# gmh14/tssplat

Hardware: NVIDIA H100
Metric: geometry_energy_grad_iters_per_sec_64x4k (higher is better)
Workload: dtype f32

## Files before the change

include/tssplat_b200.h:

```cpp
#ifndef TSSPLAT_B200_H_
#define TSSPLAT_B200_H_

#include <stdint.h>

#ifdef __cplusplus
extern "C" {
#endif

#define TSB_VERSION 2

enum {
  TSB_OK = 0,
  TSB_E_INVALID = -1,
  TSB_E_MESH = -2,
  TSB_E_CUDA = -3,
  TSB_E_NOMEM = -4
};

typedef struct tsb_handle_s *tsb_handle_t;

typedef struct {
  int32_t warps_per_cta;
  int32_t laplacian_scale;
  int32_t ring_slots;
  int32_t force_global;
  int32_t tet_cost_x100;
  int32_t enable_amips;
  int32_t reserved[2];
} tsb_options_t;

typedef struct {
  float c1, c2;
  int32_t order;
  float c3;
  int32_t reserved[4];
} tsb_terms_t;

typedef struct {
  int32_t n;
  int32_t nele;
  int32_t n_components;
  int32_t grid;
  int32_t warps_per_cta;
  int32_t ctas_per_sm;
  int32_t mode_global;
  int32_t smem_bytes;
  int32_t ring_slots;
  int32_t n_segments;
  int32_t n_boundary_faces;
  int32_t max_component_vertices;
  int64_t nnz;
  int64_t nnz_padded;
  int64_t device_bytes;
  int64_t stream_bytes;
} tsb_info_t;

int tsb_create(const float *rest_xyz, const int32_t *tets, int32_t n, int32_t nele,
               const tsb_options_t *opt, int device, tsb_handle_t *out);

void tsb_destroy(tsb_handle_t h);

const char *tsb_last_error(tsb_handle_t h);

int tsb_get_info(tsb_handle_t h, tsb_info_t *info);

int tsb_energy_grad(tsb_handle_t h, const float *x_dev, float c1, float c2, int32_t order,
                    float gradH, const float *gradH_dev, float *energy_out_dev,
                    float *grad_out_dev, void *stream);

int tsb_energy_grad_ex(tsb_handle_t h, const float *x_dev, const tsb_terms_t *terms, float gradH,
                       const float *gradH_dev, float *energy_out_dev, float *grad_out_dev, void *stream);

int tsb_energy_grad_host(tsb_handle_t h, const float *x_host, float c1, float c2, int32_t order,
                         float gradH, float *energy_out_host, float *grad_out_host, void *stream);

int tsb_scale(const float *g_dev, int64_t count, float gradH, const float *gradH_dev,
              float *out_dev, void *stream);

int tsb_grad_limit(float *grad_dev, int64_t count, float s_threshold, float s, float *work_dev, void *stream);

int tsb_adam_uniform_step(float *p_dev, const float *grad_dev, float *g1_dev, float *g2_dev,
                          int64_t count, double lr, double beta1, double beta2, int32_t step,
                          double grad_limit, float *work_dev, void *stream);

typedef struct tsb_surface_s *tsb_surface_t;
int tsb_surface_create(const int32_t *surface_vid, int32_t nsv, const int32_t *surface_f, int32_t nsf,
                       int32_t n_tet_vertices, int device, tsb_surface_t *out);
void tsb_surface_destroy(tsb_surface_t s);
const char *tsb_surface_last_error(tsb_surface_t s);
int tsb_surface_forward(tsb_surface_t s, const float *tet_v_dev, float *v_pos_dev, float *v_nrm_dev, void *stream);
int tsb_surface_backward(tsb_surface_t s, const float *tet_v_dev, const float *grad_v_pos_dev,
                         const float *grad_v_nrm_dev, float *grad_tet_v_dev, void *stream);

int tsb_surface_extract(const int32_t *tets_host, int32_t nele, int32_t n, int device, int32_t *nsv_out,
                        int32_t *nsf_out, int32_t **surface_vid_out, int32_t **surface_f_out);
void tsb_free_host(void *p);
const char *tsb_setup_last_error(void);

#ifdef __cplusplus
}
#endif
#endif
```

tssplat_b200/_capi.py:

```python
from __future__ import annotations

import ctypes as C
import os

from . import build as _build

LIB_PATH = os.environ.get("TSSPLAT_B200_LIB") or _build.LIB_PATH

TSB_OK, TSB_E_INVALID, TSB_E_MESH, TSB_E_CUDA, TSB_E_NOMEM = 0, -1, -2, -3, -4

EXPORTED_SYMBOLS = (
    "tsb_create", "tsb_destroy", "tsb_last_error", "tsb_get_info", "tsb_energy_grad", "tsb_energy_grad_ex", "tsb_energy_grad_host", "tsb_scale",
    "tsb_grad_limit", "tsb_adam_uniform_step",
    "tsb_surface_create", "tsb_surface_destroy", "tsb_surface_last_error", "tsb_surface_forward", "tsb_surface_backward",
    "tsb_surface_extract", "tsb_free_host", "tsb_setup_last_error",
)


class tsb_options_t(C.Structure):
    _fields_ = [("warps_per_cta", C.c_int32), ("laplacian_scale", C.c_int32), ("ring_slots", C.c_int32),
                ("force_global", C.c_int32), ("tet_cost_x100", C.c_int32), ("enable_amips", C.c_int32), ("reserved", C.c_int32 * 2)]


class tsb_terms_t(C.Structure):
    _fields_ = [("c1", C.c_float), ("c2", C.c_float), ("order", C.c_int32), ("c3", C.c_float), ("reserved", C.c_int32 * 4)]


class tsb_info_t(C.Structure):
    _fields_ = [
        ("n", C.c_int32), ("nele", C.c_int32), ("n_components", C.c_int32), ("grid", C.c_int32),
        ("warps_per_cta", C.c_int32), ("ctas_per_sm", C.c_int32), ("mode_global", C.c_int32),
        ("smem_bytes", C.c_int32), ("ring_slots", C.c_int32), ("n_segments", C.c_int32),
        ("n_boundary_faces", C.c_int32), ("max_component_vertices", C.c_int32),
        ("nnz", C.c_int64), ("nnz_padded", C.c_int64), ("device_bytes", C.c_int64), ("stream_bytes", C.c_int64),
    ]


def _load() -> C.CDLL:
    if not os.path.exists(LIB_PATH):
        raise ImportError(
            f"{LIB_PATH} is missing: the CUDA library has not been built "
            "(run `python -m tssplat_b200.build`); tssplat_b200 has no CPU fallback")
    try:
        lib = C.CDLL(LIB_PATH)
    except OSError as e:
        raise ImportError(f"cannot load {LIB_PATH}: {e}; tssplat_b200 has no CPU fallback") from e
    vp, f32, i32, i64 = C.c_void_p, C.c_float, C.c_int32, C.c_int64
    lib.tsb_create.restype = C.c_int
    lib.tsb_create.argtypes = [vp, vp, i32, i32, C.POINTER(tsb_options_t), C.c_int, C.POINTER(vp)]
    lib.tsb_destroy.restype = None
    lib.tsb_destroy.argtypes = [vp]
    lib.tsb_last_error.restype = C.c_char_p
    lib.tsb_last_error.argtypes = [vp]
    lib.tsb_get_info.restype = C.c_int
    lib.tsb_get_info.argtypes = [vp, C.POINTER(tsb_info_t)]
    lib.tsb_energy_grad.restype = C.c_int
    lib.tsb_energy_grad.argtypes = [vp, vp, f32, f32, i32, f32, vp, vp, vp, vp]
    lib.tsb_energy_grad_ex.restype = C.c_int
    lib.tsb_energy_grad_ex.argtypes = [vp, vp, C.POINTER(tsb_terms_t), f32, vp, vp, vp, vp]
    lib.tsb_energy_grad_host.restype = C.c_int
    lib.tsb_energy_grad_host.argtypes = [vp, vp, f32, f32, i32, f32, vp, vp, vp]
    lib.tsb_scale.restype = C.c_int
    lib.tsb_scale.argtypes = [vp, i64, f32, vp, vp, vp]
    lib.tsb_grad_limit.restype = C.c_int
    lib.tsb_grad_limit.argtypes = [vp, i64, f32, f32, vp, vp]
    lib.tsb_adam_uniform_step.restype = C.c_int
    lib.tsb_adam_uniform_step.argtypes = [vp, vp, vp, vp, i64, C.c_double, C.c_double, C.c_double, i32, C.c_double, vp, vp]
    lib.tsb_surface_create.restype = C.c_int
    lib.tsb_surface_create.argtypes = [vp, i32, vp, i32, i32, C.c_int, C.POINTER(vp)]
    lib.tsb_surface_destroy.restype = None
    lib.tsb_surface_destroy.argtypes = [vp]
    lib.tsb_surface_last_error.restype = C.c_char_p
    lib.tsb_surface_last_error.argtypes = [vp]
    lib.tsb_surface_forward.restype = C.c_int
    lib.tsb_surface_forward.argtypes = [vp, vp, vp, vp, vp]
    lib.tsb_surface_backward.restype = C.c_int
    lib.tsb_surface_backward.argtypes = [vp, vp, vp, vp, vp, vp]
    lib.tsb_surface_extract.restype = C.c_int
    lib.tsb_surface_extract.argtypes = [vp, C.c_int32, C.c_int32, C.c_int, C.POINTER(C.c_int32), C.POINTER(C.c_int32),
                                        C.POINTER(C.POINTER(C.c_int32)), C.POINTER(C.POINTER(C.c_int32))]
    lib.tsb_free_host.restype = None
    lib.tsb_free_host.argtypes = [vp]
    lib.tsb_setup_last_error.restype = C.c_char_p
    lib.tsb_setup_last_error.argtypes = []
    return lib


# ... 13 lines not shown
```

tssplat_b200/csrc/tsb_capi.cu:

```cuda
#include <cuda_runtime.h>

#include <cstdio>
#include <cstring>
#include <string>
#include <vector>

#include "../../include/tssplat_b200.h"
#include "tsb_kernels.cuh"
#include "tsb_plan.h"

struct tsb_handle_s {
  int device = 0;
  tsb::KParams kp{};
  tsb::LaunchConfig lc{};
  float *stage_x[2] = {nullptr, nullptr}, *stage_grad[2] = {nullptr, nullptr}, *stage_energy[2] = {nullptr, nullptr};
  cudaStream_t s_pipe[2] = {nullptr, nullptr};
  cudaEvent_t ev_run[2] = {nullptr, nullptr}, ev_done[2] = {nullptr, nullptr};
  unsigned host_calls = 0;
  bool amips = false;
  tsb_info_t info{};
  std::vector<void *> allocs;
  std::string err;
};

// ... 97 lines not shown
  pc.grid_cb = [&](int area_verts, bool &global_mode, int &grid, std::string &err) -> int {
    if (!global_mode) {
      int r = ring;
      while (r > 2 && tsb::energy_smem_bytes(nw, r, cpc, area_verts, false) > smem_optin) --r;
      if (tsb::energy_smem_bytes(nw, r, cpc, area_verts, false) > smem_optin) global_mode = true;
      else slots = r;
    }
    if (global_mode) while (slots > 2 && tsb::energy_smem_bytes(nw, slots, cpc, 0, true) > smem_optin) --slots;
    smem = tsb::energy_smem_bytes(nw, slots, cpc, global_mode ? 0 : area_verts, global_mode);
    int ctas = 0;
    cudaError_t e = tsb::energy_occupancy(nw, smem, global_mode, pc.enable_amips != 0, &ctas);
    if (e != cudaSuccess || ctas < 1) {
      err = std::string("kernel does not fit the device: ") + (e != cudaSuccess ? cudaGetErrorString(e) : "occupancy 0");
      return TSB_E_CUDA;
    }
    ctas_per_sm = std::min(ctas, nw == 16 ? 1 : 2);
    grid = ctas_per_sm * sms;
    return TSB_OK;
  };

  tsb::HostPlan plan;
  std::string err;
  int rc = tsb::build_plan(rest_xyz, tets, n, nele, pc, plan, err);
  if (rc != TSB_OK) return fail(nullptr, rc, err);

  tsb_handle_t h = new tsb_handle_s();
  h->device = device;
  tsb::KParams &kp = h->kp;
#define TSB_TRY(expr) do { rc = (expr); if (rc != TSB_OK) { g_create_err = h->err; tsb_destroy(h); return rc; } } while (0)
  TSB_TRY(upload(h, plan.stream, kp.stream, 16));
  TSB_TRY(upload(h, plan.X4, kp.X4, 4));
  TSB_TRY(upload(h, plan.segs, kp.segs));
  TSB_TRY(upload(h, plan.cta_seg, kp.cta_seg, 2));
  TSB_TRY(upload(h, plan.wdesc, kp.wdesc, 2));
  TSB_TRY(upload(h, plan.wseg, kp.wseg, 2));
  TSB_TRY(upload(h, plan.vlist, kp.vlist));
  TSB_TRY(upload(h, plan.pos16, kp.pos16, 2));
  TSB_TRY(upload(h, plan.pos_gid, kp.pos_gid));
  TSB_TRY(upload(h, plan.orphans, kp.orphans));
  if (pc.enable_amips) {
    TSB_TRY(upload(h, plan.Bt, kp.Bt, 4));
    TSB_TRY(upload(h, plan.wtc0, kp.wtc0));
  }
  TSB_TRY(alloc_zero(h, size_t(plan.n_components), &kp.done));
  TSB_TRY(upload(h, std::vector<unsigned long long>(size_t(plan.grid) * 4, tsb::kEnergySentinel), kp.cta_energy, 2));
#ifdef TSB_TRACE
  TSB_TRY(alloc_zero(h, size_t(plan.grid) * 16, &kp.trace));
#endif
  if (plan.mode_global) {
    TSB_TRY(alloc_zero(h, size_t(plan.n), &kp.u4g));
    TSB_TRY(alloc_zero(h, size_t(plan.n), &kp.x4g));
  }
#undef TSB_TRY
  kp.n_orphans = int32_t(plan.orphans.size());
  kp.n_components = plan.n_components;
  kp.n = plan.n;
  kp.vh = plan.vh;
  kp.ring_bytes = tsb::energy_ring_bytes(slots, cpc, plan.mode_global != 0);
  kp.cells_per_chunk = cpc;
  kp.ring_slots = slots;
  kp.stage_bytes = plan.mode_global ? 0 : plan.area_verts * 32;
  h->lc = tsb::LaunchConfig{nw, plan.grid, smem, plan.mode_global, 0};
  h->amips = pc.enable_amips != 0;

  tsb_info_t &I = h->info;
  I.n = plan.n; I.nele = plan.nele; I.n_components = plan.n_components; I.grid = plan.grid;
  I.warps_per_cta = nw; I.ctas_per_sm = ctas_per_sm; I.mode_global = plan.mode_global; I.smem_bytes = smem;
  I.ring_slots = slots; I.n_segments = int32_t(plan.segs.size()); I.n_boundary_faces = plan.n_boundary_faces;
  I.max_component_vertices = plan.max_comp_verts; I.nnz = plan.nnz; I.nnz_padded = plan.nnz_padded;
  int64_t staged = 0;
  for (const tsb::SegHdr &s : plan.segs) staged += s.nv;
  I.stream_bytes = int64_t(plan.stream.size()) + (plan.mode_global ? int64_t(plan.n) * (12 + 16 + 64) : staged * (16 + 12 + 2)) +
                   int64_t(plan.n) * 12 + int64_t(plan.segs.size()) * 32 + int64_t(plan.grid) * (16 + 8 * nw);
  *out = h;
  return TSB_OK;
}

void tsb_destroy(tsb_handle_t h) {
  if (!h) return;
  DeviceGuard guard(h->device);
  for (int k = 0; k < 2; ++k) {
    if (h->ev_run[k]) cudaEventDestroy(h->ev_run[k]);
    if (h->ev_done[k]) cudaEventDestroy(h->ev_done[k]);
    if (h->s_pipe[k]) cudaStreamDestroy(h->s_pipe[k]);
  }
  for (void *p : h->allocs) cudaFree(p);
  delete h;
}

const char *tsb_last_error(tsb_handle_t h) { return h ? h->err.c_str() : g_create_err.c_str(); }

int tsb_get_info(tsb_handle_t h, tsb_info_t *info) {
  if (!h || !info) return TSB_E_INVALID;
  *info = h->info;
  return TSB_OK;
}

static int energy_grad_impl(tsb_handle_t h, const float *x_dev, float c1, float c2, float c3, int32_t order, float gradH,
                            const float *gradH_dev, float *energy_out_dev, int energy4, float *grad_out_dev, void *stream) {
  if (!h) return TSB_E_INVALID;
  if (!x_dev || !energy_out_dev) return fail(h, TSB_E_INVALID, "x_dev and energy_out_dev must be non-null");
  if (order != 2 && order != 4)
    return fail(h, TSB_E_INVALID, "order must be 2 or 4 (the reference yields zeros for anything else: tet_spheres_cuda.cu:57-63)");
  if (c3 != 0.f && !h->amips) return fail(h, TSB_E_INVALID, "c3 != 0 needs a handle created with tsb_options_t.enable_amips = 1");
  DeviceGuard guard(h->device);
  if (!guard.ok) return fail(h, TSB_E_CUDA, "cannot select the handle's CUDA device");
  tsb::KParams kp = h->kp;
  kp.x = x_dev; kp.grad = grad_out_dev; kp.energy_out = energy_out_dev; kp.gradH_dev = gradH_dev;
  kp.c1 = c1; kp.c2 = c2; kp.c3 = c3; kp.gradH = gradH; kp.order = order; kp.energy4 = energy4;
  tsb::LaunchConfig lc = h->lc;
  lc.amips = c3 != 0.f ? 1 : 0;
  cudaError_t e = tsb::launch_energy_grad(kp, lc, static_cast<cudaStream_t>(stream));
  if (e != cudaSuccess) return fail(h, TSB_E_CUDA, std::string("energy_grad launch: ") + cudaGetErrorString(e));
  return TSB_OK;
}

int tsb_energy_grad(tsb_handle_t h, const float *x_dev, float c1, float c2, int32_t order, float gradH,
                    const float *gradH_dev, float *energy_out_dev, float *grad_out_dev, void *stream) {
  return energy_grad_impl(h, x_dev, c1, c2, 0.f, order, gradH, gradH_dev, energy_out_dev, 0, grad_out_dev, stream);
}

int tsb_energy_grad_ex(tsb_handle_t h, const float *x_dev, const tsb_terms_t *terms, float gradH, const float *gradH_dev,
                       float *energy_out_dev, float *grad_out_dev, void *stream) {
  if (!h) return TSB_E_INVALID;
  if (!terms) return fail(h, TSB_E_INVALID, "terms is null");
  return energy_grad_impl(h, x_dev, terms->c1, terms->c2, terms->c3, terms->order, gradH, gradH_dev, energy_out_dev, 1, grad_out_dev, stream);
// ... 110 lines not shown
```

tssplat_b200/csrc/tsb_kernels.cu:

```cuda
#include <cuda_runtime.h>

#include <cmath>
#include <cstdint>

#include "tsb_kernels.cuh"

namespace tsb {

namespace {

__device__ __forceinline__ double warp_sum(double v) {
#pragma unroll
  for (int o = 16; o > 0; o >>= 1) v += __shfl_xor_sync(0xffffffffu, v, o);
  return v;
}

__device__ __forceinline__ uint32_t smem_u32(const void *p) { return uint32_t(__cvta_generic_to_shared(p)); }
__device__ __forceinline__ void mbar_fence_init() { asm volatile("fence.mbarrier_init.release.cluster;" ::: "memory"); }
__device__ __forceinline__ unsigned int ld_acquire(const unsigned int *p) {
  unsigned int v;
  asm volatile("ld.acquire.gpu.global.u32 %0, [%1];" : "=r"(v) : "l"(p) : "memory");
  return v;
}

constexpr int align_up(int v, int a) { return (v + a - 1) / a * a; }
constexpr int kMaxSlots = 8;
constexpr unsigned long long kSentinel = kEnergySentinel;

#ifdef TSB_TRACE
__device__ __forceinline__ unsigned long long gtime() { unsigned long long t; asm volatile("mov.u64 %0, %%globaltimer;" : "=l"(t)); return t; }
#define TSB_STAMP(i) do { if (tid == 0 && p.trace) p.trace[blockIdx.x * 16 + (i)] = (i) == 0 ? gtime() : (unsigned long long)clock64(); } while (0)
#else
#define TSB_STAMP(i) do { } while (0)
#endif

__host__ __device__ constexpr int off_rings(int stage_bytes) { return align_up(stage_bytes, 128); }
__host__ __device__ constexpr int off_bars(int stage_bytes, int nw, int ring) { return off_rings(stage_bytes) + nw * ring; }
__host__ __device__ constexpr int off_red(int stage_bytes, int nw, int ring) { return off_bars(stage_bytes, nw, ring) + nw * kMaxSlots * 8; }
constexpr int kSegTab = 16;
__host__ __device__ constexpr int off_segtab(int stage_bytes, int nw, int ring) { return align_up(off_red(stage_bytes, nw, ring) + nw * 24, 32); }
__host__ __device__ constexpr int off_wsegtab(int stage_bytes, int nw, int ring) { return off_segtab(stage_bytes, nw, ring) + kSegTab * 32; }
__host__ __device__ constexpr int smem_total(int stage_bytes, int nw, int ring) { return align_up(off_wsegtab(stage_bytes, nw, ring) + kSegTab * nw * 4, 128); }

struct f32x2 { float lo, hi; };
__device__ __forceinline__ f32x2 pk2(float lo, float hi) { return f32x2{lo, hi}; }
__device__ __forceinline__ float sum2(f32x2 v) { return v.lo + v.hi; }
__device__ __forceinline__ void fma2_acc(f32x2 &acc, f32x2 a, f32x2 b) { acc.lo = fmaf(a.lo, b.lo, acc.lo); acc.hi = fmaf(a.hi, b.hi, acc.hi); }

__device__ __forceinline__ float rel_u(float x, float X, float c) {
  const float s = x - X, bb = s - x;
  const float e = (x - (s - bb)) + (-X - bb);
  return (s - c) + e;
}

template <bool GLOBAL> struct Fmt;
template <> struct Fmt<false> { static constexpr uint32_t CELL = kCellStaged, IB = 2, TPL = 2; };
template <> struct Fmt<true> { static constexpr uint32_t CELL = kCellGlobal, IB = 4, TPL = 1; };

template <uint32_t CELL>
struct WarpStream {
  const unsigned char *next_src;
  uint32_t bytes_left;
  uint32_t bars;
  unsigned char *ring;
  unsigned char *cell;
  uint32_t chunk_bytes, cpc, nslot;
  uint32_t cc, slot, phase, cells_left;
  int lane;

  __device__ __forceinline__ void request(uint32_t smem_dst, uint32_t bar) {
    const uint32_t bytes = min(chunk_bytes, bytes_left);
    asm volatile("mbarrier.arrive.expect_tx.shared::cta.b64 _, [%0], %1;" ::"r"(bar), "r"(bytes) : "memory");
    asm volatile("cp.async.bulk.shared::cluster.global.mbarrier::complete_tx::bytes [%0], [%1], %2, [%3];" ::"r"(smem_dst), "l"(next_src),
                 "r"(bytes), "r"(bar)
                 : "memory");
    next_src += bytes;
    bytes_left -= bytes;
  }
  __device__ __forceinline__ void wait(uint32_t bar, uint32_t parity) {
    uint32_t ok;
    do {
      asm volatile("{\n.reg .pred p;\nmbarrier.try_wait.parity.shared::cta.b64 p, [%1], %2;\nselp.u32 %0, 1, 0, p;\n}" : "=r"(ok) : "r"(bar), "r"(parity) : "memory");
    } while (!ok);
  }
  __device__ __forceinline__ void begin() {
    if (cells_left) wait(bars, 0);
  }
  __device__ __forceinline__ uint32_t avail() const { return cpc - cc; }
  __device__ __forceinline__ void advance(uint32_t n) {
    cell += n * CELL;
    cc += n;
    cells_left -= n;
    if (cc == cpc) {
      cc = 0;
      __syncwarp();
      if (lane == 0 && bytes_left) request(smem_u32(cell) - chunk_bytes, bars + slot * 8);
      if (++slot == nslot) { slot = 0; cell = ring; phase ^= 1u; }
      if (cells_left) wait(bars + slot * 8, phase);
    }
  }
};

template <int NW, int MINB, bool GLOBAL, bool AMIPS>
__global__ void __launch_bounds__(NW * 32, MINB) energy_grad_kernel(const KParams p) {
  using F = Fmt<GLOBAL>;
  constexpr int NT = NW * 32;
  constexpr uint32_t CELL = F::CELL, WOFF = 128 * F::IB;
  constexpr int SV = GLOBAL ? 1 : (1024 + NT - 1) / NT;
  extern __shared__ __align__(128) unsigned char smem[];

  const int tid = threadIdx.x, warp = tid >> 5, lane = tid & 31;
  const int ring = p.ring_bytes, stage_bytes = p.stage_bytes;
  TSB_STAMP(0); TSB_STAMP(1);
  double *red = reinterpret_cast<double *>(smem + off_red(stage_bytes, NW, ring));
  float4 *stage = reinterpret_cast<float4 *>(smem);

  const int2 cs = __ldg(&p.cta_seg[blockIdx.x]);
  WarpStream<CELL> ws;
  {
    const uint2 wd = __ldg(&p.wdesc[blockIdx.x * NW + warp]);
    ws.next_src = p.stream + size_t(wd.x) * 16;
    ws.bytes_left = wd.y;
    ws.cells_left = wd.y / CELL;
    ws.ring = smem + off_rings(stage_bytes) + warp * ring;
    ws.bars = smem_u32(smem + off_bars(stage_bytes, NW, ring)) + warp * kMaxSlots * 8;
    ws.cpc = uint32_t(p.cells_per_chunk);
    ws.chunk_bytes = ws.cpc * CELL;
    ws.nslot = uint32_t(p.ring_slots);
    ws.cell = ws.ring;
    ws.cc = 0; ws.slot = 0; ws.phase = 0; ws.lane = lane;
    if (lane == 0) {
      for (uint32_t i = 0; i < ws.nslot; ++i) asm volatile("mbarrier.init.shared::cta.b64 [%0], %1;" ::"r"(ws.bars + i * 8), "r"(1) : "memory");
      mbar_fence_init();
      for (uint32_t i = 0; i < ws.nslot && ws.bytes_left; ++i) ws.request(smem_u32(ws.ring) + i * ws.chunk_bytes, ws.bars + i * 8);
    }
    __syncwarp();
  }
  const int vh = p.vh;
  auto ubase_of = [&](const SegHdr &h, int li) -> int { return h.whole ? 0 : (li & 1) * 2 * vh; };
  auto xbase_of = [&](const SegHdr &h, int li) -> int { return h.whole ? h.npos : (li & 1) * 2 * vh + vh; };

  SegHdr *segtab = reinterpret_cast<SegHdr *>(smem + off_segtab(stage_bytes, NW, ring));
  ushort2 *wsegtab = reinterpret_cast<ushort2 *>(smem + off_wsegtab(stage_bytes, NW, ring));
  {
    const int nsc = min(cs.y - cs.x, kSegTab);
    const int4 *src = reinterpret_cast<const int4 *>(p.segs + cs.x);
    for (int i = tid; i < nsc * 2; i += NT) reinterpret_cast<int4 *>(segtab)[i] = __ldg(src + i);
    for (int i = tid; i < nsc * NW; i += NT) wsegtab[i] = __ldg(&p.wseg[size_t(cs.x) * NW + i]);
  }
  auto seg_at = [&](int s) -> SegHdr { return (s - cs.x < kSegTab) ? segtab[s - cs.x] : p.segs[s]; };
  auto wseg_at = [&](int s) -> ushort2 { return (s - cs.x < kSegTab) ? wsegtab[(s - cs.x) * NW + warp] : __ldg(&p.wseg[size_t(s) * NW + warp]); };
  SegHdr hcur{};
  float px[SV][3];
  float4 pX[SV];
  bool pre = false;
  SegHdr h1{};
  if (cs.x < cs.y) {
    hcur = p.segs[cs.x];
    if (!GLOBAL && cs.x + 1 < cs.y) h1 = p.segs[cs.x + 1];
    if (!GLOBAL && !hcur.whole) {
#pragma unroll
      for (int k = 0; k < SV; ++k) {
        const int v = tid + k * NT;
        if (v < hcur.nv) { pX[k] = __ldg(&p.X4[hcur.x4off + v]); pX[k].w = __uint_as_float(uint32_t(__ldg(&p.pos16[hcur.x4off + v]))); }
      }
    }
  }
  TSB_STAMP(2);
  asm volatile("griddepcontrol.launch_dependents;" ::: "memory");
  asm volatile("griddepcontrol.wait;" ::: "memory");
  TSB_STAMP(3);

  const float gh = p.gradH * (p.gradH_dev ? __ldcg(p.gradH_dev) : 1.f);
  const float s1 = gh * p.c1, s2 = gh * p.c2, s3 = gh * p.c3;
  const bool amips_on = AMIPS && p.c3 != 0.f && p.Bt != nullptr;
  const bool order2 = p.order == 2;
  float *__restrict__ grad = p.grad;
  if (grad) {
    for (int i = blockIdx.x * NT + tid; i < p.n_orphans; i += gridDim.x * NT) {
      const int v = __ldg(&p.orphans[i]);
      grad[3 * size_t(v)] = 0.f; grad[3 * size_t(v) + 1] = 0.f; grad[3 * size_t(v) + 2] = 0.f;
    }
  }

  double des = 0.0, deb = 0.0, dea = 0.0;

  auto load_ref = [&](const SegHdr &h, float (&r)[3]) {
    const size_t gr = size_t(h.vbase >= 0 ? h.vbase : __ldg(&p.vlist[h.x4off]));
    const float4 Xr = __ldg(&p.X4[h.x4off]);
    r[0] = __ldcg(p.x + 3 * gr) - Xr.x; r[1] = __ldcg(p.x + 3 * gr + 1) - Xr.y; r[2] = __ldcg(p.x + 3 * gr + 2) - Xr.z;
  };
  auto load_x = [&](const SegHdr &h) {
#pragma unroll
    for (int k = 0; k < SV; ++k) {
      const int v = tid + k * NT;
      if (v < h.nv) {
        const size_t gi = size_t(h.vbase >= 0 ? h.vbase + v : __ldg(&p.vlist[h.x4off + v]));
        px[k][0] = __ldcg(p.x + 3 * gi); px[k][1] = __ldcg(p.x + 3 * gi + 1); px[k][2] = __ldcg(p.x + 3 * gi + 2);
      }
    }
  };
  auto store_staged = [&](const SegHdr &h, int li) {
    float4 *ub = stage + ubase_of(h, li), *xb = stage + xbase_of(h, li);
    float pr[3];
    load_ref(h, pr);
#pragma unroll
    for (int k = 0; k < SV; ++k) {
      const int v = tid + k * NT;
      if (v < h.nv) {
        const uint32_t pos = __float_as_uint(pX[k].w);
        ub[pos] = make_float4(rel_u(px[k][0], pX[k].x, pr[0]), rel_u(px[k][1], pX[k].y, pr[1]), rel_u(px[k][2], pX[k].z, pr[2]), 0.f);
        xb[pos] = make_float4(px[k][0], px[k][1], px[k][2], 0.f);
      }
    }
  };
  auto stage_direct = [&](const SegHdr &h, int li) {
    float4 *ub = stage + ubase_of(h, li), *xb = stage + xbase_of(h, li);
    float r[3];
    load_ref(h, r);
    for (int v = tid; v < h.nv; v += NT) {
      const float4 X = __ldg(&p.X4[h.x4off + v]);
      const size_t gi = size_t(h.vbase >= 0 ? h.vbase + v : __ldg(&p.vlist[h.x4off + v]));
// ... 67 lines not shown
            if (v < hn.nv) { pX[k] = __ldg(&p.X4[hn.x4off + v]); pX[k].w = __uint_as_float(uint32_t(__ldg(&p.pos16[hn.x4off + v]))); }
          }
          load_x(hn);
        }
      }
    }

    auto gatherU = [&](uint32_t j) -> float4 { return GLOBAL ? __ldg(p.u4g + j) : *reinterpret_cast<const float4 *>(smem + j); };
    auto gatherX = [&](uint32_t j) -> float4 { return GLOBAL ? __ldg(p.x4g + j) : *reinterpret_cast<const float4 *>(smem + j); };
    const int xb16 = GLOBAL ? 0 : xbase_of(hcur, li) * 16;
    auto gid_x = [&](uint32_t j) -> size_t {
      if (GLOBAL) return size_t(j);
      return size_t(__ldg(&p.pos_gid[hcur.p4off + ((j - uint32_t(xb16)) >> 4)]));
    };
    const float4 uref = GLOBAL ? __ldg(p.u4g + hcur.x4off) : stage[ubase_of(hcur, li)];
    if (s == cs.x) TSB_STAMP(13);

    for (int rb = 0; rb < int(wseg.x); ++rb) {
      const uint32_t hdr = *reinterpret_cast<const uint32_t *>(ws.cell + WOFF + lane * 16);
      const uint32_t rid = hdr & 0xFFFFFFu, len4 = (hdr >> 24) & 63u, llog = hdr >> 30;
      const bool active = rid != 0xFFFFFFu;
      const uint32_t rowj = GLOBAL ? *reinterpret_cast<const uint32_t *>(ws.cell + lane * 16)
                                   : uint32_t(*reinterpret_cast<const uint16_t *>(ws.cell + lane * 8));
      const float4 ui = gatherU(rowj);
      f32x2 AX{0.f, 0.f}, AY{0.f, 0.f}, AZ{0.f, 0.f};
      uint32_t left = len4;
      while (left) {
        const uint32_t n = min(left, ws.avail());
        const unsigned char *cp = ws.cell + lane * 4 * F::IB;
#pragma unroll 2
        for (uint32_t q = 0; q < n; ++q, cp += CELL) {
          uint32_t j[4];
          if (GLOBAL) {
            const uint4 qi = *reinterpret_cast<const uint4 *>(cp);
            j[0] = qi.x; j[1] = qi.y; j[2] = qi.z; j[3] = qi.w;
          } else {
            const uint2 qi = *reinterpret_cast<const uint2 *>(cp);
            j[0] = qi.x & 0xFFFFu; j[1] = qi.x >> 16; j[2] = qi.y & 0xFFFFu; j[3] = qi.y >> 16;
          }
          const float4 qw = *reinterpret_cast<const float4 *>(cp + WOFF + lane * (16 - 4 * F::IB));
          const float4 u0 = gatherU(j[0]), u1 = gatherU(j[1]), u2 = gatherU(j[2]), u3 = gatherU(j[3]);
          const f32x2 W01 = pk2(qw.x, qw.y), W23 = pk2(qw.z, qw.w);
          fma2_acc(AX, W01, pk2(u0.x - ui.x, u1.x - ui.x));
          fma2_acc(AY, W01, pk2(u0.y - ui.y, u1.y - ui.y));
          fma2_acc(AZ, W01, pk2(u0.z - ui.z, u1.z - ui.z));
          fma2_acc(AX, W23, pk2(u2.x - ui.x, u3.x - ui.x));
          fma2_acc(AY, W23, pk2(u2.y - ui.y, u3.y - ui.y));
          fma2_acc(AZ, W23, pk2(u2.z - ui.z, u3.z - ui.z));
        }
        ws.advance(n);
        left -= n;
      }
#ifdef TSB_TRACE
      if (s == cs.x && rb == 0) { TSB_STAMP(14); if (tid == 0 && p.trace) p.trace[blockIdx.x * 16 + 15] = len4 | (uint32_t(wseg.x) << 16) | (uint32_t(wseg.y) << 24); }
#endif
      float ax = sum2(AX), ay = sum2(AY), az = sum2(AZ);
      for (uint32_t o = 1; o < (1u << llog); o <<= 1) {
        ax += __shfl_xor_sync(0xffffffffu, ax, o);
        ay += __shfl_xor_sync(0xffffffffu, ay, o);
        az += __shfl_xor_sync(0xffffffffu, az, o);
      }
      if (active && (lane & ((1u << llog) - 1u)) == 0) {
        des += double(fmaf(ui.x - uref.x, ax, fmaf(ui.y - uref.y, ay, (ui.z - uref.z) * az)));
        if (grad) {
          const size_t gi = rid;
          grad[3 * gi] = s1 * ax; grad[3 * gi + 1] = s1 * ay; grad[3 * gi + 2] = s1 * az;
        }
      }
    }
    if (s == cs.x) TSB_STAMP(5);
    if (grad) {
      const int bar_id = 1 + (li & 1);
      if (warp == NW - 1) {
        asm volatile("bar.sync %0, %1;" ::"r"(bar_id), "n"(NT) : "memory");
        if (lane == 0) { __threadfence(); atomicAdd(p.done + hcur.comp, 1u); }
      } else {
        asm volatile("bar.arrive %0, %1;" ::"r"(bar_id), "n"(NT) : "memory");
      }
    }

    bool waited = false;
    const int tcell0 = amips_on ? __ldg(&p.wtc0[size_t(s) * NW + warp]) : 0;
    for (int tc = 0; tc < int(wseg.y); ++tc) {
      uint32_t tj[F::TPL][4];
      float tdet[F::TPL];
      if (GLOBAL) {
        const uint4 a = *reinterpret_cast<const uint4 *>(ws.cell + lane * 16);
        tj[0][0] = a.x; tj[0][1] = a.y; tj[0][2] = a.z; tj[0][3] = a.w;
        tdet[0] = *reinterpret_cast<const float *>(ws.cell + 512 + lane * 4);
      } else {
        const uint4 a = *reinterpret_cast<const uint4 *>(ws.cell + lane * 16);
        const float2 d = *reinterpret_cast<const float2 *>(ws.cell + 512 + lane * 8);
        tj[0][0] = a.x & 0xFFFFu; tj[0][1] = a.x >> 16; tj[0][2] = a.y & 0xFFFFu; tj[0][3] = a.y >> 16;
        tj[F::TPL - 1][0] = a.z & 0xFFFFu; tj[F::TPL - 1][1] = a.z >> 16; tj[F::TPL - 1][2] = a.w & 0xFFFFu; tj[F::TPL - 1][3] = a.w >> 16;
        tdet[0] = d.x; tdet[F::TPL - 1] = d.y;
      }
      float4 xv[F::TPL][4];
#pragma unroll
      for (int t = 0; t < int(F::TPL); ++t)
#pragma unroll
        for (int k = 0; k < 4; ++k) xv[t][k] = gatherX(tj[t][k]);
      ws.advance(1);
#pragma unroll
      for (int t = 0; t < int(F::TPL); ++t) {
        const float4 x0 = xv[t][0], x1 = xv[t][1], x2 = xv[t][2], x3 = xv[t][3];
        const float idet = tdet[t];
        const float e1x = x1.x - x0.x, e1y = x1.y - x0.y, e1z = x1.z - x0.z;
// ... 64 lines not shown
              const size_t vk = 3 * gid_x(tj[t][k + 1]);
#pragma unroll
              for (int r = 0; r < 3; ++r) {
                const float g = Pm[r][0] * bb[k][0] + Pm[r][1] * bb[k][1] + Pm[r][2] * bb[k][2];
                atomicAdd(grad + vk + r, g);
                g0[r] -= g;
              }
            }
            const size_t v0 = 3 * gid_x(tj[t][0]);
            atomicAdd(grad + v0, g0[0]); atomicAdd(grad + v0 + 1, g0[1]); atomicAdd(grad + v0 + 2, g0[2]);
          }
        }
      }
    }
    if (s == cs.x) TSB_STAMP(6);

    if (s + 1 < cs.y) {
      if (!GLOBAL) {
        if (li == 0 && eager2) {
        } else {
          if (pre) {
            if (li == 1 && eager2) __syncthreads();
            store_staged(hn, li + 1);
          }
          __syncthreads();
          if (!pre) {
            stage_direct(hn, li + 1);
            __syncthreads();
          }
        }
      } else if (grad) {
        __syncthreads();
      }
    }
    hcur = hn;
  }

  TSB_STAMP(7);
  des = warp_sum(des);
  deb = warp_sum(deb);
  if (AMIPS) dea = warp_sum(dea);
  if (lane == 0) { red[3 * warp] = des; red[3 * warp + 1] = deb; red[3 * warp + 2] = dea; }
  __syncthreads();
  TSB_STAMP(8);
  if (tid == 0) {
    double a = 0.0, b = 0.0, c = 0.0;
    for (int w = 0; w < NW; ++w) { a += red[3 * w]; b += red[3 * w + 1]; c += red[3 * w + 2]; }
    a *= 0.5;
    unsigned long long ua = (unsigned long long)__double_as_longlong(a), ub = (unsigned long long)__double_as_longlong(b);
    unsigned long long uc = (unsigned long long)__double_as_longlong(c);
    if (ua == kSentinel) ua = 0x7FF8000000000000ull;
    if (ub == kSentinel) ub = 0x7FF8000000000000ull;
    if (uc == kSentinel) uc = 0x7FF8000000000000ull;
    asm volatile("st.global.v2.u64 [%0], {%1, %2};" ::"l"(p.cta_energy + 4 * blockIdx.x), "l"(ua), "l"(ub) : "memory");
    asm volatile("st.global.v2.u64 [%0], {%1, %2};" ::"l"(p.cta_energy + 4 * blockIdx.x + 2), "l"(uc), "l"(0ull) : "memory");
  }
  TSB_STAMP(9);
  if (blockIdx.x == 0 && warp == 0) {
    __syncwarp();
    double a = 0.0, b = 0.0, c3sum = 0.0;
    constexpr int kPollBatch = 5;
    for (int c0 = lane; c0 < int(gridDim.x); c0 += 32 * kPollBatch) {
      unsigned long long ua[kPollBatch], ub[kPollBatch], uc[kPollBatch], ud[kPollBatch];
      bool pending = true;
      while (pending) {
        pending = false;
#pragma unroll
        for (int k = 0; k < kPollBatch; ++k) {
          const int c = c0 + 32 * k;
          if (c < int(gridDim.x)) {
            asm volatile("ld.relaxed.gpu.global.v2.u64 {%0, %1}, [%2];" : "=l"(ua[k]), "=l"(ub[k]) : "l"(p.cta_energy + 4 * c) : "memory");
            asm volatile("ld.relaxed.gpu.global.v2.u64 {%0, %1}, [%2];" : "=l"(uc[k]), "=l"(ud[k]) : "l"(p.cta_energy + 4 * c + 2) : "memory");
          }
        }
#pragma unroll
        for (int k = 0; k < kPollBatch; ++k)
          if (c0 + 32 * k < int(gridDim.x)) pending |= ua[k] == kSentinel || ub[k] == kSentinel || uc[k] == kSentinel || ud[k] == kSentinel;
      }
#pragma unroll
      for (int k = 0; k < kPollBatch; ++k) {
        const int c = c0 + 32 * k;
        if (c < int(gridDim.x)) {
          asm volatile("st.global.v2.u64 [%0], {%1, %2};" ::"l"(p.cta_energy + 4 * c), "l"(kSentinel), "l"(kSentinel) : "memory");
          asm volatile("st.global.v2.u64 [%0], {%1, %2};" ::"l"(p.cta_energy + 4 * c + 2), "l"(kSentinel), "l"(kSentinel) : "memory");
          a += __longlong_as_double((long long)ua[k]);
          b += __longlong_as_double((long long)ub[k]);
          c3sum += __longlong_as_double((long long)uc[k]);
        }
      }
    }
    a = warp_sum(a); b = warp_sum(b); c3sum = warp_sum(c3sum);
    if (lane == 0) {
      p.energy_out[0] = float(double(p.c1) * a + double(p.c2) * b + double(p.c3) * c3sum);
      p.energy_out[1] = float(a);
      p.energy_out[2] = float(b);
      if (p.energy4) p.energy_out[3] = float(c3sum);
    }
    for (int c = lane; c < p.n_components; c += 32) p.done[c] = 0u;
  }
  TSB_STAMP(10);
#ifdef TSB_TRACE
  if (tid == 0 && p.trace) p.trace[blockIdx.x * 16 + 11] = gtime();
#endif
}

__global__ void prestage_kernel(const float *__restrict__ x, const float4 *__restrict__ X4, float4 *__restrict__ u4,
                                float4 *__restrict__ x4, int n) {
  for (int v = blockIdx.x * blockDim.x + threadIdx.x; v < n; v += gridDim.x * blockDim.x) {
    const float4 X = X4[v];
    const size_t r = size_t(__float_as_uint(X.w));
    const float4 Xr = X4[r];
    const float a = x[3 * size_t(v)], b = x[3 * size_t(v) + 1], c = x[3 * size_t(v) + 2];
    const float c0 = x[3 * r] - Xr.x, c1 = x[3 * r + 1] - Xr.y, c2 = x[3 * r + 2] - Xr.z;
    u4[v] = make_float4(rel_u(a, X.x, c0), rel_u(b, X.y, c1), rel_u(c, X.z, c2), 0.f);
    x4[v] = make_float4(a, b, c, 0.f);
  }
}

__global__ void scale_kernel(const float *__restrict__ g, int64_t count, float gradH, const float *gradH_dev,
                             float *__restrict__ out) {
  const float s = gradH * (gradH_dev ? __ldg(gradH_dev) : 1.f);
  for (int64_t i = blockIdx.x * int64_t(blockDim.x) + threadIdx.x; i < count; i += int64_t(gridDim.x) * blockDim.x)
    out[i] = s * g[i];
}

__device__ __forceinline__ void block_max_to(float v, float *dst) {
  for (int o = 16; o > 0; o >>= 1) v = fmaxf(v, __shfl_xor_sync(0xffffffffu, v, o));
  __shared__ float s_m[32];
  if ((threadIdx.x & 31) == 0) s_m[threadIdx.x >> 5] = v;
  __syncthreads();
  if (threadIdx.x < 32) {
    float m = (threadIdx.x < (blockDim.x + 31) / 32) ? s_m[threadIdx.x] : 0.f;
    for (int o = 16; o > 0; o >>= 1) m = fmaxf(m, __shfl_xor_sync(0xffffffffu, m, o));
    if (threadIdx.x == 0) atomicMax(reinterpret_cast<unsigned int *>(dst), __float_as_uint(m));
  }
  __syncthreads();
}

__global__ void absmax_kernel(const float *__restrict__ g, int64_t count, float *work) {
  float m = 0.f;
  for (int64_t i = blockIdx.x * int64_t(blockDim.x) + threadIdx.x; i < count; i += int64_t(gridDim.x) * blockDim.x)
    m = fmaxf(m, fabsf(g[i]));
  block_max_to(m, work);
}

__global__ void grad_limit_apply_kernel(float *g, int64_t count, float thr, float s, float *work) {
  const float m = __ldcg(work);
  if (m > thr) {
    const float f = s / m;
    for (int64_t i = blockIdx.x * int64_t(blockDim.x) + threadIdx.x; i < count; i += int64_t(gridDim.x) * blockDim.x) g[i] *= f;
  }
  __syncthreads();
  if (threadIdx.x == 0) {
    unsigned int *ticket = reinterpret_cast<unsigned int *>(work + 1);
    if (atomicAdd(ticket, 1u) == gridDim.x - 1) { work[0] = 0.f; *ticket = 0u; }
// ... 127 lines not shown
```

tssplat_b200/csrc/tsb_kernels.cuh:

```cuda
#pragma once
#include <cuda_runtime.h>

#include <cstdint>

#include "tsb_plan.h"

namespace tsb {

struct KParams {
  const unsigned char *stream;
  const float4 *X4;
  const int32_t *vlist;
  const uint16_t *pos16;
  const int32_t *pos_gid;
  const SegHdr *segs;
  const int2 *cta_seg;
  const uint2 *wdesc;
  const ushort2 *wseg;
  const float4 *Bt;
  const int32_t *wtc0;
  const int32_t *orphans;
  int32_t n_orphans;
  int32_t n_components;
  unsigned int *done;
  double *cta_energy;
  float4 *u4g, *x4g;
  const float *x;
  float *grad;
  float *energy_out;
  const float *gradH_dev;
  float c1, c2, c3, gradH;
  int32_t order;
  int32_t energy4;
  int32_t n;
  int32_t vh;
  int32_t ring_bytes;
  int32_t cells_per_chunk;
  int32_t ring_slots;
  int32_t stage_bytes;
#ifdef TSB_TRACE
  unsigned long long *trace;
#endif
};

struct LaunchConfig {
  int nw;
  int grid;
  int smem_bytes;
  int global;
  int amips;
};

int energy_ring_bytes(int ring_slots, int cells_per_chunk, bool global);
int energy_smem_bytes(int nw, int ring_slots, int cells_per_chunk, int area_verts, bool global);
constexpr unsigned long long kEnergySentinel = 0x7FF8F00DBAADC0DEull;
cudaError_t energy_occupancy(int nw, int smem_bytes, bool global, bool amips, int *ctas_per_sm);
cudaError_t launch_energy_grad(const KParams &p, const LaunchConfig &lc, cudaStream_t stream);

cudaError_t launch_scale(const float *g, int64_t count, float gradH, const float *gradH_dev, float *out, cudaStream_t s);
cudaError_t launch_grad_limit(float *g, int64_t count, float thr, float s, float *work4, cudaStream_t st);
cudaError_t launch_adam_uniform(float *p, const float *grad, float *g1, float *g2, int64_t count, double lr,
                                double b1, double b2, int step, double grad_limit, float *work4, cudaStream_t st);

}
```

tssplat_b200/csrc/tsb_plan.cpp:

```cpp
#include "tsb_plan.h"

#include <algorithm>
#include <atomic>
#include <cmath>
#include <cstring>
#include <numeric>
#include <thread>

#include "../../include/tssplat_b200.h"

namespace tsb {
namespace {

struct FaceKey {
  uint32_t a, b, c, owner;
  bool operator<(const FaceKey &o) const {
    if (a != o.a) return a < o.a;
    if (b != o.b) return b < o.b;
    return c < o.c;
  }
  bool same(const FaceKey &o) const { return a == o.a && b == o.b && c == o.c; }
};

const int kFace[4][3] = {{1, 2, 3}, {0, 3, 2}, {0, 1, 3}, {0, 2, 1}};
// ... 858 lines not shown
  P.wseg.assign(segs.size() * NW * 2, 0);
  std::vector<CtaStats> stats(P.grid);
  parallel_for(size_t(P.grid), 1, nth, [&](size_t b0, size_t b1) {
    for (size_t b = b0; b < b1; ++b)
      emit_cta(M, comps, segs, ring_cells, int(b), P, &wstream[b * NW], wB.empty() ? nullptr : &wB[b * NW], stats[b]);
  });
  for (const CtaStats &e : stats) {
    if (e.rc != TSB_OK) { err = e.err; return e.rc; }
    P.nnz_padded += e.nnz_padded; P.n_cells += e.n_cells; P.n_rb += e.n_rb; P.n_tetcells += e.n_tetcells;
    P.gather_wavefronts[0] += e.gwf[0]; P.gather_wavefronts[1] += e.gwf[1];
    P.tet_wavefronts[0] += e.twf[0]; P.tet_wavefronts[1] += e.twf[1];
  }
  return TSB_OK;
}

int concat_streams(const std::vector<std::vector<uint8_t>> &wstream, const std::vector<std::vector<float>> &wB, int nth,
                   HostPlan &P, std::string &err) {
  const int G = P.grid, NW = P.nw;
  if (!wB.empty()) {
    P.wtc0.assign(P.segs.size() * NW, 0);
    const size_t per_cell = size_t(3) * (P.mode_global ? 32 : 64) * 4;
    size_t cells = 0;
    for (int b = 0; b < G; ++b)
      for (int w = 0; w < NW; ++w) {
        for (int sgi = P.cta_seg[2 * size_t(b)]; sgi < P.cta_seg[2 * size_t(b) + 1]; ++sgi) {
          P.wtc0[size_t(sgi) * NW + w] = int32_t(cells);
          cells += P.wseg[(size_t(sgi) * NW + w) * 2 + 1];
        }
        const auto &v = wB[size_t(b) * NW + w];
        P.Bt.insert(P.Bt.end(), v.begin(), v.end());
      }
    if (P.Bt.size() != cells * per_cell) { err = "internal: AMIPS rest-inverse blocks out of step with the tet cells"; return TSB_E_INVALID; }
  }
  size_t total = 0;
  for (const auto &st : wstream) total += st.size();
  if (total / 16 > 0xFFFFFFFFull) { err = "plan stream exceeds 64 GiB"; return TSB_E_NOMEM; }
  P.stream.resize(std::max<size_t>(total, 16));
  P.wdesc.assign(wstream.size() * 2, 0);
  std::vector<size_t> offs(wstream.size() + 1, 0);
  for (size_t i = 0; i < wstream.size(); ++i) {
    if (wstream[i].size() > 0xFFFFFFFFull) { err = "warp stream exceeds 4 GiB"; return TSB_E_NOMEM; }
    P.wdesc[2 * i] = uint32_t(offs[i] / 16);
    P.wdesc[2 * i + 1] = uint32_t(wstream[i].size());
    offs[i + 1] = offs[i] + wstream[i].size();
  }
  uint8_t *dst = P.stream.data();
  parallel_for(wstream.size(), 16, total > (size_t(8) << 20) ? nth : 1, [&](size_t b, size_t e) {
    for (size_t i = b; i < e; ++i)
      if (!wstream[i].empty()) std::memcpy(dst + offs[i], wstream[i].data(), wstream[i].size());
  });
  return TSB_OK;
}

}

int build_plan(const float *rest, const int32_t *tets, int32_t n, int32_t nele, const PlanConfig &cfg,
               HostPlan &P, std::string &err) {
  if (!rest || !tets || n <= 0 || nele <= 0) { err = "null input or non-positive size"; return TSB_E_INVALID; }
  if (cfg.nw < 1 || cfg.nw > kMaxWarps || cfg.grid < 1) { err = "bad plan configuration"; return TSB_E_INVALID; }
  if (n >= 0xFFFFFF) { err = "more than 16.7 M vertices in one handle (row-block headers hold 24-bit row ids): shard the mesh"; return TSB_E_INVALID; }
  P = HostPlan();
  P.n = n; P.nele = nele; P.laplacian_scale = cfg.laplacian_scale ? 1 : 0;
  P.nw = cfg.nw;
  const int nth = std::clamp(int(std::thread::hardware_concurrency()), 1, kMaxHostThreads);

  int rc = validate(rest, tets, n, nele, nth, err);
  if (rc != TSB_OK) return rc;
  Mesh M{rest, tets, n, nele, std::vector<int32_t>(size_t(nele) * 4, -1), std::vector<int32_t>(size_t(n), -1), P.laplacian_scale};
  std::vector<Comp> comps = find_components(M, P);
  const bool global_mode = cfg.force_global || P.max_comp_verts > cfg.area_cap || P.max_comp_verts > kMaxStagedVerts;
  if ((rc = build_components(M, comps, global_mode, nth, P, err)) != TSB_OK) return rc;
  if ((rc = choose_layout(comps, cfg, global_mode, P, err)) != TSB_OK) return rc;
  const std::vector<Seg> segs = make_segments(comps, cut_stream(comps, double(cfg.tet_cost), P.grid), P);
  staging_tables(M, comps, segs, P);
  std::vector<std::vector<uint8_t>> wstream(size_t(P.grid) * P.nw);
  std::vector<std::vector<float>> wB(cfg.enable_amips ? wstream.size() : 0);
  if ((rc = emit_ctas(M, comps, segs, cfg.ring_cells, nth, P, wstream, wB, err)) != TSB_OK) return rc;
  return concat_streams(wstream, wB, nth, P, err);
}

}
```

tssplat_b200/csrc/tsb_plan.h:

```cpp
#pragma once
#include <cstdint>
#include <functional>
#include <memory>
#include <new>
#include <string>
#include <utility>
#include <vector>

namespace tsb {

constexpr int kCellStaged = 768, kCellGlobal = 1024;
constexpr int kMaxHalfVerts = 1023;
constexpr int kMaxStagedVerts = 2047;
constexpr int kMaxWarps = 16;
constexpr int kCellsPerChunk = 6;

struct SegHdr {
  int32_t comp;
  int32_t vbase;
  int32_t nv;
  int32_t x4off;
  int32_t expected;
  int32_t whole;
  int32_t npos;
  int32_t p4off;
};
static_assert(sizeof(SegHdr) == 32, "SegHdr must be 32 bytes");

struct PlanConfig {
  int32_t nw = 16;
  int32_t grid = 132;
  std::function<int(int area_verts, bool &global_mode, int &grid, std::string &err)> grid_cb;
  int32_t vh_cap = kMaxHalfVerts;
  int32_t area_cap = kMaxStagedVerts;
  int32_t laplacian_scale = 0;
  int32_t force_global = 0;
  float tet_cost = 3.0f;
  int32_t ring_cells = 2 * kCellsPerChunk;
  int32_t enable_amips = 0;
};

template <class T>
struct NoInitAlloc : std::allocator<T> {
  template <class U> struct rebind { using other = NoInitAlloc<U>; };
  NoInitAlloc() = default;
  template <class U> NoInitAlloc(const NoInitAlloc<U> &) {}
  template <class U> void construct(U *p) noexcept { ::new (static_cast<void *>(p)) U; }
  template <class U, class... A> void construct(U *p, A &&...a) { ::new (static_cast<void *>(p)) U(std::forward<A>(a)...); }
};

struct HostPlan {
  int32_t n = 0, nele = 0, n_components = 0, n_boundary_faces = 0, laplacian_scale = 0;
  int32_t mode_global = 0;
  int32_t nw = 0, grid = 0;
  int32_t vh = 0;
  int32_t area_verts = 0;
  int32_t max_comp_verts = 0;
  int32_t contiguous = 1;
  int64_t nnz = 0;
  int64_t nnz_padded = 0;
  int64_t n_rb = 0, n_tetcells = 0, n_cells = 0;
  int64_t gather_wavefronts[2] = {0, 0};
  int64_t tet_wavefronts[2] = {0, 0};

  std::vector<uint8_t, NoInitAlloc<uint8_t>> stream;
  std::vector<float> X4;
  std::vector<int32_t> vlist;
  std::vector<uint16_t> pos16;
  std::vector<int32_t> pos_gid;
  std::vector<SegHdr> segs;
  std::vector<int32_t> cta_seg;
  std::vector<uint32_t> wdesc;
  std::vector<uint16_t> wseg;
  std::vector<int32_t> orphans;
  std::vector<float> Bt;
  std::vector<int32_t> wtc0;
};

int build_plan(const float *rest_xyz, const int32_t *tets, int32_t n, int32_t nele,
               const PlanConfig &cfg, HostPlan &plan, std::string &err);

}
```

tssplat_b200/csrc/tsb_plan_debug.cpp:

```cpp
#include <cstring>
#include <string>

#include "../../include/tssplat_b200.h"
#include "tsb_plan.h"

struct tsbdbg_plan { tsb::HostPlan plan; };
static thread_local std::string g_err;

extern "C" {

const char *tsbdbg_last_error() { return g_err.c_str(); }

int tsbdbg_build_ex(const float *rest_xyz, const int32_t *tets, int32_t n, int32_t nele, int32_t nw, int32_t grid,
                    int32_t laplacian_scale, int32_t force_global, int32_t vh_cap, int32_t area_cap, float tet_cost,
                    int32_t ring_cells, int32_t enable_amips, tsbdbg_plan **out) {
  if (!out) return TSB_E_INVALID;
  *out = nullptr;
  tsb::PlanConfig pc;
  pc.nw = nw; pc.grid = grid; pc.laplacian_scale = laplacian_scale; pc.force_global = force_global;
  pc.enable_amips = enable_amips ? 1 : 0;
  if (vh_cap > 0) pc.vh_cap = vh_cap;
  if (area_cap > 0) pc.area_cap = area_cap;
  if (tet_cost > 0) pc.tet_cost = tet_cost;
  if (ring_cells > 0) pc.ring_cells = ring_cells;
  tsbdbg_plan *d = new tsbdbg_plan();
  const int rc = tsb::build_plan(rest_xyz, tets, n, nele, pc, d->plan, g_err);
  if (rc != TSB_OK) { delete d; return rc; }
  *out = d;
  return TSB_OK;
}

int tsbdbg_build(const float *rest_xyz, const int32_t *tets, int32_t n, int32_t nele, int32_t nw, int32_t grid,
                 int32_t laplacian_scale, int32_t force_global, int32_t vh_cap, int32_t area_cap, float tet_cost,
                 tsbdbg_plan **out) {
  return tsbdbg_build_ex(rest_xyz, tets, n, nele, nw, grid, laplacian_scale, force_global, vh_cap, area_cap, tet_cost, 0, 0, out);
}

int tsbdbg_array(tsbdbg_plan *d, const char *name, const void **ptr, int64_t *count, int32_t *elem_bytes) {
  if (!d || !name || !ptr || !count || !elem_bytes) return TSB_E_INVALID;
  const tsb::HostPlan &P = d->plan;
  const std::string k(name);
#define ARR(nm, vec, eb) if (k == nm) { *ptr = (vec).data(); *count = int64_t((vec).size()) * int64_t(sizeof((vec)[0])) / (eb); *elem_bytes = (eb); return TSB_OK; }
  ARR("stream", P.stream, 1) ARR("X4", P.X4, 4) ARR("vlist", P.vlist, 4) ARR("segs", P.segs, 4) ARR("cta_seg", P.cta_seg, 4)
  ARR("wdesc", P.wdesc, 4) ARR("wseg", P.wseg, 2) ARR("orphans", P.orphans, 4) ARR("pos16", P.pos16, 2) ARR("pos_gid", P.pos_gid, 4)
  ARR("Bt", P.Bt, 4) ARR("wtc0", P.wtc0, 4)
#undef ARR
  return TSB_E_INVALID;
}

int tsbdbg_scalars(tsbdbg_plan *d, int64_t *out16) {
  if (!d || !out16) return TSB_E_INVALID;
  const tsb::HostPlan &P = d->plan;
  const int64_t v[20] = {P.n, P.nele, P.n_components, P.n_boundary_faces, P.laplacian_scale, P.mode_global, P.nw, P.grid,
                         P.vh, P.area_verts, P.max_comp_verts, P.contiguous, P.nnz, P.nnz_padded, P.n_rb, P.n_tetcells,
                         P.gather_wavefronts[0], P.gather_wavefronts[1], P.tet_wavefronts[0], P.tet_wavefronts[1]};
  std::memcpy(out16, v, sizeof(v));
  return TSB_OK;
}

void tsbdbg_free(tsbdbg_plan *d) { delete d; }

}
```

Baseline: 67910.

## Use idle trailing CTAs to prefetch stream prefixes into L2

Trailing CTAs that own no segments become prefetch CTAs. The CTA index is rotated so these CTAs are scheduled first, and they issue cp.async.bulk.prefetch.L2 for the leading bytes of every working warp's stream. The griddepcontrol.launch_dependents call is moved to the start of the kernel so the next launch can begin overlapping earlier. The intent is to hide DRAM latency on the first stream reads, at the cost of extra L2 traffic and a possible earlier start of the dependent kernel competing for resources.

```diff
diff --git a/include/tssplat_b200.h b/include/tssplat_b200.h
--- a/include/tssplat_b200.h
+++ b/include/tssplat_b200.h
@@ -53,6 +53,9 @@
   int64_t nnz_padded;
   int64_t device_bytes;
   int64_t stream_bytes;
+  int64_t prefetch_bytes;
+  int32_t prefetch_ctas;
+  int32_t reserved;
 } tsb_info_t;
 
 int tsb_create(const float *rest_xyz, const int32_t *tets, int32_t n, int32_t nele,
diff --git a/tssplat_b200/_capi.py b/tssplat_b200/_capi.py
--- a/tssplat_b200/_capi.py
+++ b/tssplat_b200/_capi.py
@@ -33,6 +33,7 @@
         ("smem_bytes", C.c_int32), ("ring_slots", C.c_int32), ("n_segments", C.c_int32),
         ("n_boundary_faces", C.c_int32), ("max_component_vertices", C.c_int32),
         ("nnz", C.c_int64), ("nnz_padded", C.c_int64), ("device_bytes", C.c_int64), ("stream_bytes", C.c_int64),
+        ("prefetch_bytes", C.c_int64), ("prefetch_ctas", C.c_int32), ("reserved", C.c_int32),
     ]
 
 
diff --git a/tssplat_b200/csrc/tsb_capi.cu b/tssplat_b200/csrc/tsb_capi.cu
--- a/tssplat_b200/csrc/tsb_capi.cu
+++ b/tssplat_b200/csrc/tsb_capi.cu
@@ -173,6 +173,8 @@
     TSB_TRY(alloc_zero(h, size_t(plan.n), &kp.x4g));
   }
 #undef TSB_TRY
+  kp.n_prefetch = plan.n_prefetch;
+  kp.prefetch_prefix = plan.prefetch_prefix;
   kp.n_orphans = int32_t(plan.orphans.size());
   kp.n_components = plan.n_components;
   kp.n = plan.n;
@@ -193,6 +195,9 @@
   for (const tsb::SegHdr &s : plan.segs) staged += s.nv;
   I.stream_bytes = int64_t(plan.stream.size()) + (plan.mode_global ? int64_t(plan.n) * (12 + 16 + 64) : staged * (16 + 12 + 2)) +
                    int64_t(plan.n) * 12 + int64_t(plan.segs.size()) * 32 + int64_t(plan.grid) * (16 + 8 * nw);
+  I.prefetch_ctas = plan.n_prefetch;
+  if (plan.n_prefetch > 0)
+    for (size_t i = 1; i < size_t(plan.grid - plan.n_prefetch) * nw * 2; i += 2) I.prefetch_bytes += std::min(plan.wdesc[i], plan.prefetch_prefix);
   *out = h;
   return TSB_OK;
 }
diff --git a/tssplat_b200/csrc/tsb_kernels.cu b/tssplat_b200/csrc/tsb_kernels.cu
--- a/tssplat_b200/csrc/tsb_kernels.cu
+++ b/tssplat_b200/csrc/tsb_kernels.cu
@@ -29,7 +29,7 @@
 
 #ifdef TSB_TRACE
 __device__ __forceinline__ unsigned long long gtime() { unsigned long long t; asm volatile("mov.u64 %0, %%globaltimer;" : "=l"(t)); return t; }
-#define TSB_STAMP(i) do { if (tid == 0 && p.trace) p.trace[blockIdx.x * 16 + (i)] = (i) == 0 ? gtime() : (unsigned long long)clock64(); } while (0)
+#define TSB_STAMP(i) do { if (tid == 0 && p.trace) p.trace[cta * 16 + (i)] = (i) == 0 ? gtime() : (unsigned long long)clock64(); } while (0)
 #else
 #define TSB_STAMP(i) do { } while (0)
 #endif
@@ -111,14 +111,25 @@
 
   const int tid = threadIdx.x, warp = tid >> 5, lane = tid & 31;
   const int ring = p.ring_bytes, stage_bytes = p.stage_bytes;
+  const int cta = p.n_prefetch ? int((blockIdx.x + gridDim.x - unsigned(p.n_prefetch)) % gridDim.x) : int(blockIdx.x);
+  asm volatile("griddepcontrol.launch_dependents;" ::: "memory");
   TSB_STAMP(0); TSB_STAMP(1);
   double *red = reinterpret_cast<double *>(smem + off_red(stage_bytes, NW, ring));
   float4 *stage = reinterpret_cast<float4 *>(smem);
 
-  const int2 cs = __ldg(&p.cta_seg[blockIdx.x]);
+  if (cta >= int(gridDim.x) - p.n_prefetch) {
+    const int i = cta - (int(gridDim.x) - p.n_prefetch), nwk = (int(gridDim.x) - p.n_prefetch) * NW;
+    const int w1 = int(int64_t(i + 1) * nwk / p.n_prefetch);
+    for (int w = int(int64_t(i) * nwk / p.n_prefetch) + tid; w < w1; w += NT) {
+      const uint2 wd = __ldg(&p.wdesc[w]);
+      const uint32_t bytes = min(wd.y, p.prefetch_prefix);
+      if (bytes) asm volatile("cp.async.bulk.prefetch.L2.global [%0], %1;" ::"l"(p.stream + size_t(wd.x) * 16), "r"(bytes) : "memory");
+    }
+  }
+  const int2 cs = __ldg(&p.cta_seg[cta]);
   WarpStream<CELL> ws;
   {
-    const uint2 wd = __ldg(&p.wdesc[blockIdx.x * NW + warp]);
+    const uint2 wd = __ldg(&p.wdesc[cta * NW + warp]);
     ws.next_src = p.stream + size_t(wd.x) * 16;
     ws.bytes_left = wd.y;
     ws.cells_left = wd.y / CELL;
@@ -167,7 +178,6 @@
     }
   }
   TSB_STAMP(2);
-  asm volatile("griddepcontrol.launch_dependents;" ::: "memory");
   asm volatile("griddepcontrol.wait;" ::: "memory");
   TSB_STAMP(3);
 
@@ -341,7 +351,7 @@
         left -= n;
       }
 #ifdef TSB_TRACE
-      if (s == cs.x && rb == 0) { TSB_STAMP(14); if (tid == 0 && p.trace) p.trace[blockIdx.x * 16 + 15] = len4 | (uint32_t(wseg.x) << 16) | (uint32_t(wseg.y) << 24); }
+      if (s == cs.x && rb == 0) { TSB_STAMP(14); if (tid == 0 && p.trace) p.trace[cta * 16 + 15] = len4 | (uint32_t(wseg.x) << 16) | (uint32_t(wseg.y) << 24); }
 #endif
       float ax = sum2(AX), ay = sum2(AY), az = sum2(AZ);
       for (uint32_t o = 1; o < (1u << llog); o <<= 1) {
@@ -512,11 +522,11 @@
     if (ua == kSentinel) ua = 0x7FF8000000000000ull;
     if (ub == kSentinel) ub = 0x7FF8000000000000ull;
     if (uc == kSentinel) uc = 0x7FF8000000000000ull;
-    asm volatile("st.global.v2.u64 [%0], {%1, %2};" ::"l"(p.cta_energy + 4 * blockIdx.x), "l"(ua), "l"(ub) : "memory");
-    asm volatile("st.global.v2.u64 [%0], {%1, %2};" ::"l"(p.cta_energy + 4 * blockIdx.x + 2), "l"(uc), "l"(0ull) : "memory");
+    asm volatile("st.global.v2.u64 [%0], {%1, %2};" ::"l"(p.cta_energy + 4 * cta), "l"(ua), "l"(ub) : "memory");
+    asm volatile("st.global.v2.u64 [%0], {%1, %2};" ::"l"(p.cta_energy + 4 * cta + 2), "l"(uc), "l"(0ull) : "memory");
   }
   TSB_STAMP(9);
-  if (blockIdx.x == 0 && warp == 0) {
+  if (cta == 0 && warp == 0) {
     __syncwarp();
     double a = 0.0, b = 0.0, c3sum = 0.0;
     constexpr int kPollBatch = 5;
@@ -560,7 +570,7 @@
   }
   TSB_STAMP(10);
 #ifdef TSB_TRACE
-  if (tid == 0 && p.trace) p.trace[blockIdx.x * 16 + 11] = gtime();
+  if (tid == 0 && p.trace) p.trace[cta * 16 + 11] = gtime();
 #endif
 }
 
diff --git a/tssplat_b200/csrc/tsb_kernels.cuh b/tssplat_b200/csrc/tsb_kernels.cuh
--- a/tssplat_b200/csrc/tsb_kernels.cuh
+++ b/tssplat_b200/csrc/tsb_kernels.cuh
@@ -20,6 +20,8 @@
   const float4 *Bt;
   const int32_t *wtc0;
   const int32_t *orphans;
+  int32_t n_prefetch;
+  uint32_t prefetch_prefix;
   int32_t n_orphans;
   int32_t n_components;
   unsigned int *done;
diff --git a/tssplat_b200/csrc/tsb_plan.cpp b/tssplat_b200/csrc/tsb_plan.cpp
--- a/tssplat_b200/csrc/tsb_plan.cpp
+++ b/tssplat_b200/csrc/tsb_plan.cpp
@@ -934,6 +934,18 @@
   return TSB_OK;
 }
 
+void prefetch_plan(HostPlan &P) {
+  int np = 0;
+  while (np < P.grid && P.cta_seg[2 * size_t(P.grid - 1 - np)] == P.cta_seg[2 * size_t(P.grid - 1 - np) + 1]) ++np;
+  P.n_prefetch = np;
+  P.prefetch_prefix = 0;
+  if (np == 0 || np == P.grid) return;
+  uint32_t longest = 0;
+  for (size_t i = 1; i < P.wdesc.size(); i += 2) longest = std::max(longest, P.wdesc[i]);
+  const int64_t prefix = kPrefetchBytesPerCta * np / (int64_t(P.grid - np) * P.nw) / 16 * 16;
+  P.prefetch_prefix = uint32_t(std::min<int64_t>(prefix, longest));
+}
+
 }
 
 int build_plan(const float *rest, const int32_t *tets, int32_t n, int32_t nele, const PlanConfig &cfg,
@@ -958,7 +970,9 @@
   std::vector<std::vector<uint8_t>> wstream(size_t(P.grid) * P.nw);
   std::vector<std::vector<float>> wB(cfg.enable_amips ? wstream.size() : 0);
   if ((rc = emit_ctas(M, comps, segs, cfg.ring_cells, nth, P, wstream, wB, err)) != TSB_OK) return rc;
-  return concat_streams(wstream, wB, nth, P, err);
-}
-
-}
+  if ((rc = concat_streams(wstream, wB, nth, P, err)) != TSB_OK) return rc;
+  prefetch_plan(P);
+  return TSB_OK;
+}
+
+}
diff --git a/tssplat_b200/csrc/tsb_plan.h b/tssplat_b200/csrc/tsb_plan.h
--- a/tssplat_b200/csrc/tsb_plan.h
+++ b/tssplat_b200/csrc/tsb_plan.h
@@ -14,6 +14,7 @@
 constexpr int kMaxStagedVerts = 2047;
 constexpr int kMaxWarps = 16;
 constexpr int kCellsPerChunk = 6;
+constexpr int64_t kPrefetchBytesPerCta = 1024 * 1024;
 
 struct SegHdr {
   int32_t comp;
@@ -75,6 +76,8 @@
   std::vector<int32_t> orphans;
   std::vector<float> Bt;
   std::vector<int32_t> wtc0;
+  int32_t n_prefetch = 0;
+  uint32_t prefetch_prefix = 0;
 };
 
 int build_plan(const float *rest_xyz, const int32_t *tets, int32_t n, int32_t nele,
diff --git a/tssplat_b200/csrc/tsb_plan_debug.cpp b/tssplat_b200/csrc/tsb_plan_debug.cpp
--- a/tssplat_b200/csrc/tsb_plan_debug.cpp
+++ b/tssplat_b200/csrc/tsb_plan_debug.cpp
@@ -4,7 +4,7 @@
 #include "../../include/tssplat_b200.h"
 #include "tsb_plan.h"
 
-struct tsbdbg_plan { tsb::HostPlan plan; };
+struct tsbdbg_plan { tsb::HostPlan plan; uint32_t prefetch[2]; };
 static thread_local std::string g_err;
 
 extern "C" {
@@ -45,6 +45,11 @@
   ARR("wdesc", P.wdesc, 4) ARR("wseg", P.wseg, 2) ARR("orphans", P.orphans, 4) ARR("pos16", P.pos16, 2) ARR("pos_gid", P.pos_gid, 4)
   ARR("Bt", P.Bt, 4) ARR("wtc0", P.wtc0, 4)
 #undef ARR
+  if (k == "prefetch") {
+    d->prefetch[0] = uint32_t(P.n_prefetch); d->prefetch[1] = P.prefetch_prefix;
+    *ptr = d->prefetch; *count = 2; *elem_bytes = 4;
+    return TSB_OK;
+  }
   return TSB_E_INVALID;
 }
 
```

After: 73540 (median of 6 runs). +8.3%, better.
